# ZephirFXEC/HNanoSolver

Measured on AMD Instinct MI355X. Metric: solver substeps/sec (advect + 50 red-black SOR iterations + project) at N active voxels, higher is better.
Workload: dtype f32

## Files before the change

hnanosolver_amd/csrc/hns_advect.hip:

```cpp
#include <cstdlib>
#include <cstring>

#include "hns_device.hpp"

namespace hns {

struct Taps {
	int t[8];
	float fx, fy, fz;
};

constexpr unsigned kOutside = 0xFFFFE000u;
constexpr uint64_t kNarrowBytes = 0xFFFF0000ull;

__device__ __forceinline__ f3 ldv(const v4i& r, unsigned o4) {
	const v3f v = hns_buffer_load_v3f32(r, (int)(o4 + (o4 << 1)), 0, 0);
	return f3{v.x, v.y, v.z};
}
__device__ __forceinline__ float lds1(const v4i& r, unsigned o4) { return hns_buffer_load_f32(r, (int)o4, 0, 0); }

__device__ __forceinline__ void ld_zpair(const v4i& r, unsigned lo, unsigned hi, float& a, float& b) {
	const v2f32 v = hns_buffer_load_v2f32(r, (int)lo, 0, 0);
	a = v.x;
	b = v.y;
	if (hi != lo + 4u) b = lds1(r, hi);
}

struct GenericTabs {
	int nbr[27], base[27];
	__device__ __forceinline__ void set(int t, int nb) { nbr[t] = nb, base[t] = nb < 0 ? -1 : nb * 512; }
};
constexpr int kPadTab = 48;
struct NarrowTabs {
	int nbr[27];
	unsigned b4[27], b4p[kPadTab];
	__device__ __forceinline__ void set(int t, int nb) {
		const int ax = t / 9, ay = (t - 9 * ax) / 3, az = t - 9 * ax - 3 * ay;
		nbr[t] = nb, b4[t] = b4p[(ax * 4 + ay) * 4 + az] = nb < 0 ? kOutside : (unsigned)nb * 2048u;
	}
};

__device__ __forceinline__ int3 voxel_ijk(const int4 org, int n) { return int3{org.x + (n >> 6), org.y + ((n >> 3) & 7), org.z + (n & 7)}; }

template <class Tabs>
struct LeafVoxel {
	Tabs& tabs;
	const int n, leaf, idx;
	int4 org;
	int3 c;
	float px, py, pz;
	__device__ __forceinline__ LeafVoxel(const GridDev& g, Tabs& t) : tabs(t), n(threadIdx.x), leaf(launch_leaf(g, blockIdx.x)), idx(leaf * 512 + n) {}
	__device__ __forceinline__ void stage(const GridDev& g) {
		org = g.origins[leaf];
		if (threadIdx.x < 27) tabs.set(threadIdx.x, g.nbr27[leaf * 27 + threadIdx.x]);
		__syncthreads();
		c = voxel_ijk(org, n);
		px = (float)c.x, py = (float)c.y, pz = (float)c.z;
	}
};
typedef LeafVoxel<GenericTabs> GenericCtx;
typedef LeafVoxel<NarrowTabs> NarrowCtx;

__device__ __forceinline__ constexpr int tap_of(int q) { return ((q & 1) << 2) | (q & 2) | (q >> 2); }
template <int XS = 100, int YS = 10>
__device__ __forceinline__ constexpr int box_corner(int q) { return (q & 1) * XS + ((q >> 1) & 1) * YS + (q >> 2); }
__device__ __forceinline__ void tri_weights(float tx, float ty, float tz, float (&w)[8]) {
	const float itx = 1.0f - tx, ity = 1.0f - ty, itz = 1.0f - tz;
	const float w00 = itx * ity, w10 = tx * ity, w01 = itx * ty, w11 = tx * ty;
	w[0] = w00 * itz, w[1] = w10 * itz, w[2] = w01 * itz, w[3] = w11 * itz, w[4] = w00 * tz, w[5] = w10 * tz, w[6] = w01 * tz, w[7] = w11 * tz;
}
template <class T>
__device__ __forceinline__ T bfecc_limit(T phiOrig, const T (&nbr)[6], T phiForward, T phiCorr) {
	T mn = phiOrig, mx = phiOrig;
#pragma unroll
	for (int d = 0; d < 6; ++d) {
		mn = __builtin_elementwise_min(mn, nbr[d]);
		mx = __builtin_elementwise_max(mx, nbr[d]);
	}
	mn = __builtin_elementwise_min(mn, phiForward);
	mx = __builtin_elementwise_max(mx, phiForward);
	return __builtin_elementwise_max(mn, __builtin_elementwise_min(phiCorr, mx));
}
template <class Fetch>
__device__ __forceinline__ f3 bfecc_limit_v(const f3& vo, const f3& vf, const f3& vb, Fetch nbr) {
	float nx[6], ny[6], nz[6];
#pragma unroll
	for (int d = 0; d < 6; ++d) {
		const f3 t = nbr(d);
		nx[d] = t.x, ny[d] = t.y, nz[d] = t.z;
	}
	return f3{bfecc_limit(vo.x, nx, vf.x, vf.x + 0.5f * (vo.x - vb.x)), bfecc_limit(vo.y, ny, vf.y, vf.y + 0.5f * (vo.y - vb.y)),
	          bfecc_limit(vo.z, nz, vf.z, vf.z + 0.5f * (vo.z - vb.z))};
}

struct TapsB {
	unsigned o[8];
	float fx, fy, fz;
};

__device__ __forceinline__ Taps make_taps(const GridDev& g, const GenericCtx& C, float x, float y, float z) {
	Taps T;
	const int4 org = C.org;
	const int i = __float2int_rd(x), j = __float2int_rd(y), k = __float2int_rd(z);
	T.fx = x - (float)i;
	T.fy = y - (float)j;
	T.fz = z - (float)k;
	const int ax0 = (i >> 3) - (org.x >> 3) + 1, ax1 = ((i + 1) >> 3) - (org.x >> 3) + 1;
	const int ay0 = (j >> 3) - (org.y >> 3) + 1, ay1 = ((j + 1) >> 3) - (org.y >> 3) + 1;
	const int az0 = (k >> 3) - (org.z >> 3) + 1, az1 = ((k + 1) >> 3) - (org.z >> 3) + 1;
	const bool near = ((unsigned)ax0 <= 2u) & ((unsigned)ax1 <= 2u) & ((unsigned)ay0 <= 2u) & ((unsigned)ay1 <= 2u) & ((unsigned)az0 <= 2u) &
	                  ((unsigned)az1 <= 2u);
	if (near) {
		const int sx[2] = {ax0 * 9, ax1 * 9}, sy[2] = {ay0 * 3, ay1 * 3}, sz[2] = {az0, az1};
		const int lx[2] = {(i & 7) << 6, ((i + 1) & 7) << 6}, ly[2] = {(j & 7) << 3, ((j + 1) & 7) << 3}, lz[2] = {k & 7, (k + 1) & 7};
#pragma unroll
		for (int c = 0; c < 8; ++c) {
			const int di = c >> 2, dj = (c >> 1) & 1, dk = c & 1;
			const int b = C.tabs.base[sx[di] + sy[dj] + sz[dk]];
			T.t[c] = b < 0 ? -1 : b + (lx[di] | ly[dj] | lz[dk]);
		}
	} else {
		int any = 0;
		far_cell_taps(g, C.tabs.nbr, org, i, j, k, T.t);
#pragma unroll
		for (int c = 0; c < 8; ++c) any |= T.t[c];
		if (any < 0 && g.far_flag) *g.far_flag = 1;
	}
	return T;
}

__device__ __forceinline__ TapsB make_taps_b(const GridDev& g, const NarrowCtx& C, float x, float y, float z) {
	TapsB T;
	const int4 org = C.org;
	const int i = __float2int_rd(x), j = __float2int_rd(y), k = __float2int_rd(z);
	T.fx = x - (float)i;
	T.fy = y - (float)j;
	T.fz = z - (float)k;
	const unsigned dx = (unsigned)(i - (org.x - 8)), dy = (unsigned)(j - (org.y - 8)), dz = (unsigned)(k - (org.z - 8));
	if (max(dx, max(dy, dz)) < 23u) {
		const unsigned ex = dx + 1u, ey = dy + 1u, ez = dz + 1u;
		const unsigned X[2] = {(dx & 24u) << 3, (ex & 24u) << 3}, Y[2] = {(dy & 24u) << 1, (ey & 24u) << 1}, Z[2] = {(dz & 24u) >> 1, (ez & 24u) >> 1};
		const unsigned lx[2] = {(dx & 7u) << 8, (ex & 7u) << 8}, ly[2] = {(dy & 7u) << 5, (ey & 7u) << 5}, lz[2] = {(dz & 7u) << 2, (ez & 7u) << 2};
		const unsigned XY[4] = {X[0] | Y[0], X[0] | Y[1], X[1] | Y[0], X[1] | Y[1]};
		const unsigned lxy[4] = {lx[0] | ly[0], lx[0] | ly[1], lx[1] | ly[0], lx[1] | ly[1]};
		const char* tab = reinterpret_cast<const char*>(C.tabs.b4p);
#pragma unroll
		for (int c = 0; c < 8; ++c) {
			const int dij = c >> 1, dk = c & 1;
			T.o[c] = *reinterpret_cast<const unsigned*>(tab + (XY[dij] | Z[dk])) + lxy[dij] + lz[dk];
		}
	} else {
		int any = 0, ft[8];
		far_cell_taps(g, C.tabs.nbr, org, i, j, k, ft);
#pragma unroll
		for (int c = 0; c < 8; ++c) {
			any |= ft[c];
			T.o[c] = ft[c] < 0 ? kOutside : (unsigned)ft[c] << 2;
		}
		if (any < 0 && g.far_flag) *g.far_flag = 1;
	}
	return T;
}

__device__ __forceinline__ float ldz(const float* __restrict__ f, int idx) {
	const float v = f[idx < 0 ? 0 : idx];
	return idx < 0 ? 0.0f : v;
}

__device__ __forceinline__ float tri_f_t(const float* __restrict__ f, const Taps& T) {
	float c[8];
#pragma unroll
	for (int q = 0; q < 8; ++q) c[q] = ldz(f, T.t[q]);
	return tri_nest(c, T.fx, T.fy, T.fz, lerp_f);
}

__device__ __forceinline__ f3 tri_v_t(const float* __restrict__ u, const Taps& T) {
	float x[8], y[8], z[8];
#pragma unroll
	for (int q = 0; q < 8; ++q) {
		const f3 c = ld3z(u, T.t[q]);
		x[q] = c.x, y[q] = c.y, z[q] = c.z;
	}
	return f3{tri_nest(x, T.fx, T.fy, T.fz, lerp_c), tri_nest(y, T.fx, T.fy, T.fz, lerp_c), tri_nest(z, T.fx, T.fy, T.fz, lerp_c)};
}

struct V3 {
	v2f32 xy;
	float z;
};
__device__ __forceinline__ V3 lerp_v3(const V3& a, const V3& b, float w) {
	V3 r;
	r.xy = __builtin_elementwise_fma(v2f32{w, w}, b.xy - a.xy, a.xy);
	r.z = __fmaf_rn(w, b.z - a.z, a.z);
	return r;
}
__device__ __forceinline__ f3 tri_v_b(const v4i& ru, const TapsB& T) {
	V3 c[8];
#pragma unroll
	for (int q = 0; q < 8; ++q) {
		const v3f v = hns_buffer_load_v3f32(ru, (int)(T.o[q] + (T.o[q] << 1)), 0, 0);
		c[q].xy = v2f32{v.x, v.y};
		c[q].z = v.z;
	}
	const V3 r = tri_nest(c, T.fx, T.fy, T.fz, lerp_v3);
	return f3{r.xy.x, r.xy.y, r.z};
}

__device__ __forceinline__ float tri_f_b(const v4i& rf, const TapsB& T) {
	float c[8];
#pragma unroll
	for (int q = 0; q < 8; ++q) c[q] = lds1(rf, T.o[q]);
	return tri_nest(c, T.fx, T.fy, T.fz, lerp_f);
}

template <int AXIS, int DIR>
__device__ __forceinline__ int nbr_idx(const int* s_base, int leaf, int n) {
	constexpr int shift = AXIS == 0 ? 6 : (AXIS == 1 ? 3 : 0);
	constexpr int stride = 1 << shift;
	constexpr int dslot = AXIS == 0 ? 9 : (AXIS == 1 ? 3 : 1);
	const int c = (n >> shift) & 7;
	const bool inside = DIR > 0 ? c != 7 : c != 0;
	const int b = s_base[13 + DIR * dslot];
	const int in_leaf = leaf * 512 + n + DIR * stride;
	const int out_leaf = b < 0 ? -1 : b + n - DIR * 7 * stride;
	return inside ? in_leaf : out_leaf;
}

__device__ __forceinline__ void nbr6(const int* s_base, int leaf, int n, int (&t)[6]) {
	t[0] = nbr_idx<0, -1>(s_base, leaf, n);
	t[1] = nbr_idx<0, 1>(s_base, leaf, n);
	t[2] = nbr_idx<1, -1>(s_base, leaf, n);
	t[3] = nbr_idx<1, 1>(s_base, leaf, n);
	t[4] = nbr_idx<2, -1>(s_base, leaf, n);
	t[5] = nbr_idx<2, 1>(s_base, leaf, n);
}


__device__ __forceinline__ unsigned halo_off(const unsigned* s_b4, int h) {
	int slot, local;
	halo_entry(h, slot, local);
	return s_b4[slot] + ((unsigned)local << 2);
}

constexpr int kBox = 1000, kBoxShell = kBox - 512;
constexpr int kVY = 24, kVX = 10 * kVY, kVP = 10 * kVX;
template <int XS = 100, int YS = 10>
__device__ __forceinline__ void box_shell_entry(int h, int& slot, int& local, int& cell) {
	int bx, by, bz;
	if (h < 200) {
		const int side = h >= 100, r = h - 100 * side;
		bx = 9 * side, by = r / 10, bz = r - 10 * by;
	} else if (h < 360) {
		const int q = h - 200, side = q >= 80, r = q - 80 * side;
		bx = 1 + r / 10, by = 9 * side, bz = r - 10 * (bx - 1);
	} else {
		const int q = h - 360, side = q >> 6, r = q & 63;
		bx = 1 + (r >> 3), by = 1 + (r & 7), bz = 9 * side;
	}
	slot = ((bx + 7) >> 3) * 9 + ((by + 7) >> 3) * 3 + ((bz + 7) >> 3);
	local = (((bx + 7) & 7) << 6) | (((by + 7) & 7) << 3) | ((bz + 7) & 7);
	cell = bx * XS + by * YS + bz;
}
template <int XS = 100, int YS = 10>
__device__ __forceinline__ unsigned box_shell_off(const unsigned* s_b4, int h, int& cell) {
	unsigned off = 0u;
	cell = 0;
	if (h < kBoxShell) {
		int slot, local;
		box_shell_entry<XS, YS>(h, slot, local, cell);
		off = s_b4[slot] + ((unsigned)local << 2);
	}
	return off;
}
template <int XS = 100, int YS = 10>
__device__ __forceinline__ int box_own(int n) { return ((n >> 6) + 1) * XS + (((n >> 3) & 7) + 1) * YS + (n & 7) + 1; }
template <int XS = 100, int YS = 10>
__device__ __forceinline__ constexpr int box_nbr(int d) { return (d & 1 ? 1 : -1) * (d < 2 ? XS : (d < 4 ? YS : 1)); }

template <int XS, int YS, int PS>
__device__ __forceinline__ f3 velocity_box_load(float* s_box, const v4i& ru, int n, const f3& vo, unsigned off) {
	const int ob = box_own<XS, YS>(n);
	s_box[ob] = vo.x, s_box[ob + PS] = vo.y, s_box[ob + 2 * PS] = vo.z;
	f3 h = {0.0f, 0.0f, 0.0f};
	if (n < kBoxShell) h = ldv(ru, off);
	return h;
}
template <int PS>
__device__ __forceinline__ void velocity_box_store(float* s_box, int n, int cell, const f3& h) {
	if (n < kBoxShell) s_box[cell] = h.x, s_box[cell + PS] = h.y, s_box[cell + 2 * PS] = h.z;
}
__device__ __forceinline__ V3 box_v3(const float* s_box, int a) {
	V3 r;
	r.xy = v2f32{s_box[a], s_box[a + kVP]};
	r.z = s_box[a + 2 * kVP];
	return r;
}
__device__ __forceinline__ f3 box_f3(const float* s_box, int a) {
	const V3 t = box_v3(s_box, a);
	return f3{t.xy.x, t.xy.y, t.z};
}
__device__ __forceinline__ f3 tri_v_box(const float* s_box, int a, float fx, float fy, float fz) {
	V3 c[8];
#pragma unroll
	for (int q = 0; q < 8; ++q) c[q] = box_v3(s_box, a + box_corner<kVX, kVY>(tap_of(q)));
	const V3 r = tri_nest(c, fx, fy, fz, lerp_v3);
	return f3{r.xy.x, r.xy.y, r.z};
}
__device__ __forceinline__ f3 sample_velocity(const GridDev& g, const NarrowCtx& C, const v4i& ru, const float* s_box, float sx, float sy, float sz) {
	const int i = __float2int_rd(sx), j = __float2int_rd(sy), k = __float2int_rd(sz);
	const unsigned rx = (unsigned)(i - (C.org.x - 1)), ry = (unsigned)(j - (C.org.y - 1)), rz = (unsigned)(k - (C.org.z - 1));
	if (__all(max(rx, max(ry, rz)) <= 8u)) return tri_v_box(s_box, (int)(rx * (unsigned)kVX + ry * (unsigned)kVY + rz), sx - (float)i, sy - (float)j, sz - (float)k);
	return tri_v_b(ru, make_taps_b(g, C, sx, sy, sz));
}

__device__ __forceinline__ float sdf_box_load(float* s_sdf, const v4i& rs, int n, int ob, float own, unsigned off) {
	s_sdf[ob] = own;
	float h = 0.0f;
	if (n < kBoxShell) h = lds1(rs, off);
	return h;
}
__device__ __forceinline__ void sdf_box_store(float* s_sdf, int n, int cell, float h) {
	if (n < kBoxShell) s_sdf[cell] = h;
}
template <int XS, int YS>
__device__ __forceinline__ float tri_f_box(const float* s_f, int a, float fx, float fy, float fz) {
	float c[8];
#pragma unroll
	for (int q = 0; q < 8; ++q) c[q] = s_f[a + box_corner<XS, YS>(tap_of(q))];
	return tri_nest(c, fx, fy, fz, lerp_f);
}
template <int XS, int YS>
__device__ __forceinline__ f3 collide_velocity(const float* s_sdf, int ob, f3 vc, float inv_dx) {
	const float sv = s_sdf[ob];
	if (sv < 0.0f) {
		vc.x = vc.y = vc.z = 0.0f;
	} else if (sv < 0.1f) {
		float nb[6];
#pragma unroll
		for (int d = 0; d < 6; ++d) nb[d] = s_sdf[ob + box_nbr<XS, YS>(d)];
		vc = no_slip_blend(vc, sdf_normal_of(nb, inv_dx), 1.0f - (sv / 1.5f));
	}
	return vc;
}

template <bool COLL>
__device__ __forceinline__ void advect_vector_n(const GridDev& g, const float* __restrict__ u, float* __restrict__ out, const float* __restrict__ sdf, float* s_sdf, const float scaled_dt,
                                                const float inv_dx) {
	__shared__ NarrowTabs tabs;
	__shared__ float s_box[3 * kVP];
	NarrowCtx C(g, tabs);
	const v4i ru = field_rsrc(u, (unsigned)g.n_leaves * 6144u);
	const f3 vo = ldv(ru, (unsigned)C.idx << 2);
	v4i rs = {0, 0, 0, 0};
	float so = 0.0f;
	if constexpr (COLL) {
		rs = field_rsrc(sdf, (unsigned)g.n_leaves * 2048u);
		so = lds1(rs, (unsigned)C.idx << 2);
	}
	C.stage(g);
	int cell;
	const unsigned off = box_shell_off<kVX, kVY>(tabs.b4, C.n, cell);
	const int ob = box_own<kVX, kVY>(C.n);
	const f3 hv = velocity_box_load<kVX, kVY, kVP>(s_box, ru, C.n, vo, off);
	if constexpr (COLL) sdf_box_store(s_sdf, C.n, cell, sdf_box_load(s_sdf, rs, C.n, ob, so, off));
	velocity_box_store<kVP>(s_box, C.n, cell, hv);
	float sx = C.px - scaled_dt * vo.x, sy = C.py - scaled_dt * vo.y, sz = C.pz - scaled_dt * vo.z;
	float rx = C.px, ry = C.py, rz = C.pz;
	f3 vf = {0.0f, 0.0f, 0.0f}, vb = {0.0f, 0.0f, 0.0f};
	__syncthreads();
#pragma unroll 1
	for (int pass = 0; pass < 2; ++pass) {
		f3 v;
		if constexpr (COLL) {
			const int i = __float2int_rd(sx), j = __float2int_rd(sy), k = __float2int_rd(sz);
			const unsigned cx = (unsigned)(i - (C.org.x - 1)), cy = (unsigned)(j - (C.org.y - 1)), cz = (unsigned)(k - (C.org.z - 1));
			const bool boxed = __all(max(cx, max(cy, cz)) <= 8u);
			const int a = (int)(cx * (unsigned)kVX + cy * (unsigned)kVY + cz);
			float d;
			if (boxed)
				d = tri_f_box<kVX, kVY>(s_sdf, a, sx - (float)i, sy - (float)j, sz - (float)k);
			else
				d = tri_f_b(rs, make_taps_b(g, C, sx, sy, sz));
			if (d < 0.0f) sx = rx, sy = ry, sz = rz;
			v = sample_velocity(g, C, ru, s_box, sx, sy, sz);
		} else {
			v = sample_velocity(g, C, ru, s_box, sx, sy, sz);
		}
		if (pass == 0) {
			vf = v;
			if constexpr (COLL) rx = sx, ry = sy, rz = sz;
			sx = sx + scaled_dt * v.x, sy = sy + scaled_dt * v.y, sz = sz + scaled_dt * v.z;
		} else {
			vb = v;
		}
	}
	f3 vc = bfecc_limit_v(vo, vf, vb, [&](int d) { return box_f3(s_box, ob + box_nbr<kVX, kVY>(d)); });
	if constexpr (COLL) vc = collide_velocity<kVX, kVY>(s_sdf, ob, vc, inv_dx);
	st3(out, C.idx, vc);
}
__global__ __launch_bounds__(512) __attribute__((amdgpu_waves_per_eu(8, 8))) void k_advect_vector_n(const GridDev g, const float* __restrict__ u, float* __restrict__ out, const float scaled_dt) {
	advect_vector_n<false>(g, u, out, nullptr, nullptr, scaled_dt, 0.0f);
}
constexpr int kVectorCollLds = (3 * kVP + kVP) * 4 + (int)sizeof(NarrowTabs);
static_assert(kVectorCollLds <= 160 * 1024 / 4, "k_advect_vector_n<true>: four workgroups per CU no longer fit the LDS");
template <bool COLL>
__global__ __launch_bounds__(512) __attribute__((amdgpu_waves_per_eu(8, 8))) void k_advect_vector_n(const GridDev g, const float* __restrict__ u, float* __restrict__ out,
                                                                                                const float* __restrict__ sdf, const float scaled_dt, const float inv_dx) {
	static_assert(COLL, "without a collision field: the kernel of the same name that takes no SDF");
	__shared__ float s_sdf[kVP];
	advect_vector_n<true>(g, u, out, sdf, s_sdf, scaled_dt, inv_dx);
}

template <bool COLL>
__global__ __launch_bounds__(512) void k_advect_vector(const GridDev g, const float* __restrict__ u, float* __restrict__ out,
                                                       const float* __restrict__ sdf, const float scaled_dt, const float inv_dx) {
	__shared__ GenericTabs tabs;
	GenericCtx C(g, tabs);
	C.stage(g);
	const int idx = C.idx;

	const f3 vo = ld3(u, idx);
	float sx = C.px - scaled_dt * vo.x, sy = C.py - scaled_dt * vo.y, sz = C.pz - scaled_dt * vo.z;
	float rx = C.px, ry = C.py, rz = C.pz;
	f3 vf = {0.0f, 0.0f, 0.0f}, vb = {0.0f, 0.0f, 0.0f};
#pragma unroll 1
	for (int pass = 0; pass < 2; ++pass) {
		Taps T = make_taps(g, C, sx, sy, sz);
		if (COLL) {
			if (tri_f_t(sdf, T) < 0.0f) {
				sx = rx, sy = ry, sz = rz;
				T = make_taps(g, C, sx, sy, sz);
			}
		}
		const f3 v = tri_v_t(u, T);
		if (pass == 0) {
			vf = v;
			rx = sx, ry = sy, rz = sz;
			sx = sx + scaled_dt * v.x, sy = sy + scaled_dt * v.y, sz = sz + scaled_dt * v.z;
		} else {
			vb = v;
		}
	}
	int nb[6];
	nbr6(tabs.base, C.leaf, C.n, nb);
	f3 vc = bfecc_limit_v(vo, vf, vb, [&](int d) { return ld3z(u, nb[d]); });

	if (COLL) {
		const float sv = sdf[idx];
		if (sv < 0.0f) {
			vc.x = vc.y = vc.z = 0.0f;
		} else if (sv < 0.1f) {
			const f3 nrm = sdf_normal(g, tabs.nbr, C.org, sdf, C.c.x, C.c.y, C.c.z, inv_dx);
			vc = no_slip_blend(vc, nrm, 1.0f - (sv / 1.5f));
		}
	}
	st3(out, idx, vc);
}


__global__ __launch_bounds__(512) void k_advect_scalar_n(const GridDev g, const float* __restrict__ u, const float* __restrict__ in, float* __restrict__ out,
                                                         const float scaled_dt) {
	__shared__ NarrowTabs tabs;
	NarrowCtx C(g, tabs);
	C.stage(g);
	const int n = C.n;
	const unsigned bytes1 = (unsigned)g.n_leaves * 2048u, own = (unsigned)C.idx << 2;
	const v4i ru = field_rsrc(u, bytes1 * 3u), rf = field_rsrc(in, bytes1);

	__shared__ float s_tile[kTile];
	const float phiOrig = lds1(rf, own);
	s_tile[n] = phiOrig;
	if (n < 384) s_tile[512 + n] = lds1(rf, halo_off(tabs.b4, n));
	const f3 vc = ldv(ru, own);
	float sx = C.px - scaled_dt * vc.x, sy = C.py - scaled_dt * vc.y, sz = C.pz - scaled_dt * vc.z;
	float phiForward = 0.0f, phiBackward = 0.0f;
#pragma unroll 1
	for (int pass = 0; pass < 2; ++pass) {
		const TapsB T = make_taps_b(g, C, sx, sy, sz);
		const float phi = tri_f_b(rf, T);
		if (pass == 0) {
			phiForward = phi;
			const f3 vf = tri_v_b(ru, T);
			sx = sx + scaled_dt * vf.x, sy = sy + scaled_dt * vf.y, sz = sz + scaled_dt * vf.z;
		} else {
			phiBackward = phi;
		}
	}
	const float error = phiOrig - phiBackward;
	__syncthreads();
	const float nv[6] = {s_tile[tile_nbr<0, -1>(n)], s_tile[tile_nbr<0, 1>(n)], s_tile[tile_nbr<1, -1>(n)], s_tile[tile_nbr<1, 1>(n)], s_tile[tile_nbr<2, -1>(n)], s_tile[tile_nbr<2, 1>(n)]};
	out[C.idx] = bfecc_limit(phiOrig, nv, phiForward, phiForward + 0.5f * error);
}

template <bool COLL>
__global__ __launch_bounds__(512) void k_advect_scalar(const GridDev g, const float* __restrict__ u, const float* __restrict__ in,
                                                       float* __restrict__ out, const float* __restrict__ sdf, const float scaled_dt) {
	__shared__ GenericTabs tabs;
	GenericCtx C(g, tabs);
	C.stage(g);
	const int idx = C.idx;

	const float phiOrig = in[idx];
	const f3 vc = ld3(u, idx);
	float sx = C.px - scaled_dt * vc.x, sy = C.py - scaled_dt * vc.y, sz = C.pz - scaled_dt * vc.z;
	float rx = C.px, ry = C.py, rz = C.pz;
	float phiForward = 0.0f, phiBackward = 0.0f;
#pragma unroll 1
	for (int pass = 0; pass < 2; ++pass) {
		Taps T = make_taps(g, C, sx, sy, sz);
		if (COLL) {
			if (tri_f_t(sdf, T) < 0.0f) {
				sx = rx, sy = ry, sz = rz;
				T = make_taps(g, C, sx, sy, sz);
			}
		}
		const float phi = tri_f_t(in, T);
		if (pass == 0) {
			phiForward = phi;
			const f3 vf = tri_v_t(u, T);
			rx = sx, ry = sy, rz = sz;
			sx = sx + scaled_dt * vf.x, sy = sy + scaled_dt * vf.y, sz = sz + scaled_dt * vf.z;
		} else {
			phiBackward = phi;
		}
	}
	const float error = phiOrig - phiBackward;
	int nb[6];
	nbr6(tabs.base, C.leaf, C.n, nb);
	float nv[6];
#pragma unroll
	for (int d = 0; d < 6; ++d) nv[d] = ldz(in, nb[d]);
	out[idx] = bfecc_limit(phiOrig, nv, phiForward, phiForward + 0.5f * error);
}


#define HNS_MAX_SCALARS 8
struct ScalarPtrs {
	const float* in[HNS_MAX_SCALARS];
	float* out[HNS_MAX_SCALARS];
	int n;
	const float* q4;
	float* q4_out[4];
};

__device__ __forceinline__ float tri_f_zpair(const v4i& rf, const TapsB& T) {
	float c[8];
#pragma unroll
	for (int m = 0; m < 4; ++m) ld_zpair(rf, T.o[2 * m], T.o[2 * m + 1], c[2 * m], c[2 * m + 1]);
	return tri_nest(c, T.fx, T.fy, T.fz, lerp_f);
}
__global__ __launch_bounds__(512) __attribute__((amdgpu_waves_per_eu(8, 8))) void k_advect_scalar_multi_n(const GridDev g, const float* __restrict__ u, const ScalarPtrs P, const float scaled_dt) {
	__shared__ NarrowTabs tabs;
	NarrowCtx C(g, tabs);
	const int n = C.n;
	const unsigned bytes1 = (unsigned)g.n_leaves * 2048u, own = (unsigned)C.idx << 2;
	const v4i ru = field_rsrc(u, bytes1 * 3u);
	const f3 vc = ldv(ru, own);
	C.stage(g);
	float sx = C.px - scaled_dt * vc.x, sy = C.py - scaled_dt * vc.y, sz = C.pz - scaled_dt * vc.z;
	TapsB B, F;
#pragma unroll 1
	for (int pass = 0; pass < 2; ++pass) {
		F = make_taps_b(g, C, sx, sy, sz);
		if (pass == 0) {
			B = F;
			const f3 vf = tri_v_b(ru, B);
			sx = sx + scaled_dt * vf.x, sy = sy + scaled_dt * vf.y, sz = sz + scaled_dt * vf.z;
		}
	}
	const unsigned ho = n < 384 ? halo_off(tabs.b4, n) : 0u;
	__shared__ float s_tile[2][kTile];
	for (int s = 0; s < P.n; ++s) {
		const v4i rf = field_rsrc(P.in[s], bytes1);
		float* tile = s_tile[s & 1];
		const float phiOrig = lds1(rf, own);
		tile[n] = phiOrig;
		if (n < 384) tile[512 + n] = lds1(rf, ho);
		const float phiForward = tri_f_zpair(rf, B), phiBackward = tri_f_zpair(rf, F);
		const float error = phiOrig - phiBackward;
		__syncthreads();
		const float nv[6] = {tile[tile_nbr<0, -1>(n)], tile[tile_nbr<0, 1>(n)], tile[tile_nbr<1, -1>(n)], tile[tile_nbr<1, 1>(n)], tile[tile_nbr<2, -1>(n)], tile[tile_nbr<2, 1>(n)]};
		P.out[s][C.idx] = bfecc_limit(phiOrig, nv, phiForward, phiForward + 0.5f * error);
	}
}

__device__ __forceinline__ void interp_from_taps(const Taps& T, int oob, int (&ix)[8], float (&w)[8]) {
	tri_weights(T.fx, T.fy, T.fz, w);
#pragma unroll
	for (int q = 0; q < 8; ++q) ix[q] = T.t[tap_of(q)] < 0 ? oob : T.t[tap_of(q)];
}
__device__ __forceinline__ void add_weighted(f3& a, const f3& v, float w) { a.x = a.x + w * v.x, a.y = a.y + w * v.y, a.z = a.z + w * v.z; }

template <bool BOX>
__device__ __forceinline__ bool sample_setup(const GridDev& g, const NarrowCtx& C, float x, float y, float z, unsigned oob4, int& cell, unsigned (&o)[8], float (&w)[8]) {
	const int i = __float2int_rd(x), j = __float2int_rd(y), k = __float2int_rd(z);
	const unsigned rx = (unsigned)(i - (C.org.x - 1)), ry = (unsigned)(j - (C.org.y - 1)), rz = (unsigned)(k - (C.org.z - 1));
	const bool boxed = BOX && max(rx, max(ry, rz)) <= 8u;
	cell = boxed ? (int)((rx * 10u + ry) * 10u + rz) : 0;
	float tx, ty, tz;
	if (boxed) {
		tx = x - (float)i, ty = y - (float)j, tz = z - (float)k;
#pragma unroll
		for (int q = 0; q < 8; ++q) o[q] = 0u;
	} else {
		const TapsB T = make_taps_b(g, C, x, y, z);
		tx = T.fx, ty = T.fy, tz = T.fz;
#pragma unroll
		for (int q = 0; q < 8; ++q) o[q] = T.o[tap_of(q)] >= kOutside ? oob4 : T.o[tap_of(q)];
	}
	tri_weights(tx, ty, tz, w);
	return boxed;
}

__device__ __forceinline__ bool sdf_hit(const GridDev& g, const NarrowCtx& C, const v4i& rs, const float* s_sdf, float x, float y, float z) {
	const int i = __float2int_rd(x), j = __float2int_rd(y), k = __float2int_rd(z);
	const unsigned rx = (unsigned)(i - (C.org.x - 1)), ry = (unsigned)(j - (C.org.y - 1)), rz = (unsigned)(k - (C.org.z - 1));
	float d;
	if (max(rx, max(ry, rz)) <= 8u)
		d = tri_f_box<100, 10>(s_sdf, (int)((rx * 10u + ry) * 10u + rz), x - (float)i, y - (float)j, z - (float)k);
	else
		d = tri_f_b(rs, make_taps_b(g, C, x, y, z));
	return d < 0.0f;
}
template <bool Q4, bool AHEAD, bool COLL>
__device__ __forceinline__ void advect_scalars_n(const GridDev& g, const float* __restrict__ u, const ScalarPtrs& P, const float scaled_dt, float* __restrict__ adv_out,
                                                 const float* __restrict__ sdf) {
	static_assert(!(Q4 && AHEAD), "the look-ahead form is float-only");
	static_assert(!(AHEAD && COLL), "with a collider the next substep rewrites the velocity before it advects it: nothing to look ahead to");
	__shared__ NarrowTabs tabs;
	NarrowCtx C(g, tabs);
	const int n = C.n, idx = C.idx;
	const unsigned bytes1 = (unsigned)g.n_leaves * 2048u;
	const v4i ru = field_rsrc(u, bytes1 * 3u);
	const unsigned own = (unsigned)idx << 2, oob4 = (unsigned)g.oob << 2;
	const f3 vc = ldv(ru, own);
	v4i rs = {0, 0, 0, 0};
	float so = 0.0f;
	if constexpr (COLL) {
		rs = field_rsrc(sdf, bytes1);
		so = lds1(rs, own);
	}
	C.stage(g);

	const int ob = box_own(n);
	int hcell;
	unsigned ho = box_shell_off(tabs.b4, n, hcell);
	__shared__ float s_sdf[COLL ? kBox : 1];
	if constexpr (COLL) sdf_box_store(s_sdf, n, hcell, sdf_box_load(s_sdf, rs, n, ob, so, ho));
	ho = ho >= kOutside ? oob4 : ho;
	constexpr bool FIRST = Q4;
	__shared__ float s_ubox[FIRST ? 3 * kBox : 1];
	if constexpr (FIRST) velocity_box_store<kBox>(s_ubox, n, hcell, velocity_box_load<100, 10, kBox>(s_ubox, ru, n, vc, ho));

	float bx = C.px - scaled_dt * vc.x, by = C.py - scaled_dt * vc.y, bz = C.pz - scaled_dt * vc.z;
	__shared__ float s_back[COLL && FIRST ? 3 * 512 : 1];
	if constexpr (COLL) {
		__syncthreads();
		if (sdf_hit(g, C, rs, s_sdf, bx, by, bz)) bx = C.px, by = C.py, bz = C.pz;
		if constexpr (FIRST) s_back[n] = bx, s_back[n + 512] = by, s_back[n + 1024] = bz;
		asm volatile("" : "+v"(bx), "+v"(by), "+v"(bz));
	}
	unsigned bo[8], fo[8];
	float bw[8], fw[8];
	bool bboxed = false;
	int ba = 0;
	f3 vf = {0.0f, 0.0f, 0.0f};
	__shared__ float s_vbox[AHEAD ? 3 * kVP : 1];
	__shared__ float s_wf[AHEAD ? 3 * 512 : 1];
	if constexpr (AHEAD) {
		int vcell;
		const unsigned voff = box_shell_off<kVX, kVY>(tabs.b4, n, vcell);
		const f3 hv = velocity_box_load<kVX, kVY, kVP>(s_vbox, ru, n, vc, voff);
		const TapsB T = make_taps_b(g, C, bx, by, bz);
		V3 c[8];
#pragma unroll
		for (int q = 0; q < 8; ++q) {
			const v3f v = hns_buffer_load_v3f32(ru, (int)(T.o[tap_of(q)] + (T.o[tap_of(q)] << 1)), 0, 0);
			c[tap_of(q)].xy = v2f32{v.x, v.y};
			c[tap_of(q)].z = v.z;
		}
		const float* __restrict__ uoob = u + 3 * (size_t)g.oob;
		const f3 uo = {uoob[0], uoob[1], uoob[2]};
		velocity_box_store<kVP>(s_vbox, n, vcell, hv);
		tri_weights(T.fx, T.fy, T.fz, bw);
		V3 z[4];
#pragma unroll
		for (int q = 0; q < 8; ++q) {
			const int t = tap_of(q);
			const bool outside = T.o[t] >= kOutside;
			bo[q] = outside ? oob4 : T.o[t];
			add_weighted(vf, f3{outside ? uo.x : c[t].xy.x, outside ? uo.y : c[t].xy.y, outside ? uo.z : c[t].z}, bw[q]);
			if (t & 1) z[t >> 1] = lerp_v3(c[t - 1], c[t], T.fz);
		}
		const V3 r = tri_nest_yx(z, T.fx, T.fy, lerp_v3);
		s_wf[n] = r.xy.x, s_wf[n + 512] = r.xy.y, s_wf[n + 1024] = r.z;
	} else {
		bboxed = sample_setup<FIRST>(g, C, bx, by, bz, oob4, ba, bo, bw);
		f3 vt[8];
		if (!bboxed) {
#pragma unroll
			for (int q = 0; q < 8; ++q) vt[q] = ldv(ru, bo[q]);
		}
		if constexpr (FIRST && !COLL) __syncthreads();
		if (bboxed) {
#pragma unroll
			for (int q = 0; q < 8; ++q) {
				const int a = ba + box_corner(q);
				vt[q] = f3{s_ubox[a], s_ubox[a + kBox], s_ubox[a + 2 * kBox]};
			}
		}
#pragma unroll
		for (int q = 0; q < 8; ++q) add_weighted(vf, vt[q], bw[q]);
	}
	int fa;
	float fx = bx + scaled_dt * vf.x, fy = by + scaled_dt * vf.y, fz = bz + scaled_dt * vf.z;
	if constexpr (COLL) {
		if (sdf_hit(g, C, rs, s_sdf, fx, fy, fz)) {
			if constexpr (FIRST) {
				int m = n;
				asm volatile("" : "+v"(m));
				fx = s_back[m], fy = s_back[m + 512], fz = s_back[m + 1024];
			} else {
				fx = bx, fy = by, fz = bz;
			}
		}
	}
	const bool boxed = sample_setup<true>(g, C, fx, fy, fz, oob4, fa, fo, fw);
	constexpr bool SHARE = COLL && Q4;
	if constexpr (SHARE) {
		if (bboxed) bo[0] = (unsigned)ba;
		if (boxed) fo[0] = (unsigned)fa;
		asm volatile("" : "+v"(bo[0]), "+v"(fo[0]));
	}
	const int bcell = SHARE ? (int)bo[0] : ba, fcell = SHARE ? (int)fo[0] : fa;
	__shared__ float s_box[2][kBox];
	if constexpr (Q4) {
		__shared__ v4f32 s_box4[kBox];
		const v4i rq = field_rsrc(P.q4, bytes1 * 4u);
		const v4f32 phiOrig = hns_buffer_load_v4f32(rq, (int)(own << 2), 0, 0);
		s_box4[ob] = phiOrig;
		if (n < kBoxShell) s_box4[hcell] = hns_buffer_load_v4f32(rq, (int)(ho << 2), 0, 0);
		v4f32 phiF = {0.0f, 0.0f, 0.0f, 0.0f}, phiB = {0.0f, 0.0f, 0.0f, 0.0f};
		if (!bboxed) {
			v4f32 c[8];
#pragma unroll
			for (int q = 0; q < 8; ++q) c[q] = hns_buffer_load_v4f32(rq, (int)(bo[q] << 2), 0, 0);
#pragma unroll
			for (int q = 0; q < 8; ++q) phiF = __builtin_elementwise_fma(c[q], v4f32{bw[q], bw[q], bw[q], bw[q]}, phiF);
		}
		if (!boxed) {
			v4f32 c[8];
#pragma unroll
			for (int q = 0; q < 8; ++q) c[q] = hns_buffer_load_v4f32(rq, (int)(fo[q] << 2), 0, 0);
#pragma unroll
			for (int q = 0; q < 8; ++q) phiB = __builtin_elementwise_fma(c[q], v4f32{fw[q], fw[q], fw[q], fw[q]}, phiB);
		}
		__syncthreads();
		if (bboxed) {
#pragma unroll
			for (int q = 0; q < 8; ++q) phiF = __builtin_elementwise_fma(s_box4[bcell + box_corner(q)], v4f32{bw[q], bw[q], bw[q], bw[q]}, phiF);
		}
		if (boxed) {
#pragma unroll
			for (int q = 0; q < 8; ++q) phiB = __builtin_elementwise_fma(s_box4[fcell + box_corner(q)], v4f32{fw[q], fw[q], fw[q], fw[q]}, phiB);
		}
		v4f32 nv[6];
#pragma unroll
		for (int d = 0; d < 6; ++d) nv[d] = s_box4[ob + box_nbr(d)];
		const v4f32 r = bfecc_limit(phiOrig, nv, phiF, __builtin_elementwise_fma(v4f32{0.5f, 0.5f, 0.5f, 0.5f}, phiOrig - phiB, phiF));
		P.q4_out[0][idx] = r.x, P.q4_out[1][idx] = r.y, P.q4_out[2][idx] = r.z, P.q4_out[3][idx] = r.w;
	}
	for (int s = 0; s < P.n; ++s) {
		const v4i rf = field_rsrc(P.in[s], bytes1);
		float* box = s_box[s & 1];
		const float phiOrig = lds1(rf, own);
		box[ob] = phiOrig;
		if (n < kBoxShell) box[hcell] = lds1(rf, ho);
		float vb[8], vf8[8];
		if (!bboxed) {
#pragma unroll
			for (int q = 0; q < 4; ++q) ld_zpair(rf, bo[q], bo[q + 4], vb[q], vb[q + 4]);
		}
		if (!boxed) {
#pragma unroll
			for (int q = 0; q < 4; ++q) ld_zpair(rf, fo[q], fo[q + 4], vf8[q], vf8[q + 4]);
		}
		float phiF = 0.0f, phiB = 0.0f;
		__syncthreads();
		if (bboxed) {
#pragma unroll
			for (int q = 0; q < 8; ++q) vb[q] = box[bcell + box_corner(q)];
		}
#pragma unroll
		for (int q = 0; q < 8; ++q) phiF = __fmaf_rn(vb[q], bw[q], phiF);
		if (boxed) {
#pragma unroll
			for (int q = 0; q < 8; ++q) vf8[q] = box[fcell + box_corner(q)];
		}
#pragma unroll
		for (int q = 0; q < 8; ++q) phiB = __fmaf_rn(vf8[q], fw[q], phiB);
		float nv[6];
#pragma unroll
		for (int d = 0; d < 6; ++d) nv[d] = box[ob + box_nbr(d)];
		P.out[s][idx] = bfecc_limit(phiOrig, nv, phiF, __fmaf_rn(0.5f, phiOrig - phiB, phiF));
	}
	if constexpr (AHEAD) {
		__syncthreads();
		int m = n;
		asm volatile("" : "+v"(m));
		const int obv = box_own<kVX, kVY>(m);
		const int3 w = voxel_ijk(C.org, m);
		const f3 vo = box_f3(s_vbox, obv);
		const f3 wf = f3{s_wf[m], s_wf[m + 512], s_wf[m + 1024]};
		const float cx = (float)w.x - scaled_dt * vo.x, cy = (float)w.y - scaled_dt * vo.y, cz = (float)w.z - scaled_dt * vo.z;
		const f3 wb = sample_velocity(g, C, ru, s_vbox, cx + scaled_dt * wf.x, cy + scaled_dt * wf.y, cz + scaled_dt * wf.z);
		st3(adv_out, idx, bfecc_limit_v(vo, wf, wb, [&](int d) { return box_f3(s_vbox, obv + box_nbr<kVX, kVY>(d)); }));
	}
}

template <bool Q4, bool AHEAD = false>
__global__ __launch_bounds__(512) __attribute__((amdgpu_waves_per_eu(Q4 || AHEAD ? 6 : 4))) void k_advect_scalars_n(const GridDev g, const float* __restrict__ u, const ScalarPtrs P, const float scaled_dt,
                                                                                                            float* __restrict__ adv_out) {
	advect_scalars_n<Q4, AHEAD, false>(g, u, P, scaled_dt, adv_out, nullptr);
}
constexpr int kScalarsQ4CollLds = (int)sizeof(NarrowTabs) + (3 * kBox + 2 * kBox + 4 * kBox + kBox + 3 * 512) * 4;
static_assert(kScalarsQ4CollLds <= 160 * 1024 / 3, "k_advect_scalars_n<true, false, true>: three workgroups per CU no longer fit the LDS");
template <bool Q4, bool AHEAD, bool COLL>
__global__ __launch_bounds__(512) __attribute__((amdgpu_waves_per_eu(Q4 ? 6 : 4))) void k_advect_scalars_n(const GridDev g, const float* __restrict__ u, const ScalarPtrs P, const float* __restrict__ sdf,
                                                                                                   const float scaled_dt) {
	static_assert(COLL && !AHEAD, "without a collision field: the kernel of the same name that takes no SDF");
	advect_scalars_n<Q4, false, true>(g, u, P, scaled_dt, nullptr, sdf);
}

template <bool COLL>
__global__ __launch_bounds__(512) void k_advect_scalars(const GridDev g, const float* __restrict__ u, const ScalarPtrs P,
                                                        const float* __restrict__ sdf, const float scaled_dt) {
	__shared__ GenericTabs tabs;
	GenericCtx C(g, tabs);
	C.stage(g);
	const int idx = C.idx;

	const f3 vc = ld3(u, idx);
	float sx = C.px - scaled_dt * vc.x, sy = C.py - scaled_dt * vc.y, sz = C.pz - scaled_dt * vc.z;
	float rx = C.px, ry = C.py, rz = C.pz;
	int bi[8], fi[8];
	float bw[8], fw[8];
#pragma unroll 1
	for (int pass = 0; pass < 2; ++pass) {
		Taps T = make_taps(g, C, sx, sy, sz);
		if (COLL) {
			if (tri_f_t(sdf, T) < 0.0f) {
				sx = rx, sy = ry, sz = rz;
				T = make_taps(g, C, sx, sy, sz);
			}
		}
		if (pass == 0) {
			interp_from_taps(T, g.oob, bi, bw);
			f3 vf = {0.0f, 0.0f, 0.0f};
#pragma unroll
			for (int q = 0; q < 8; ++q) add_weighted(vf, ld3(u, bi[q]), bw[q]);
			rx = sx, ry = sy, rz = sz;
			sx = sx + scaled_dt * vf.x, sy = sy + scaled_dt * vf.y, sz = sz + scaled_dt * vf.z;
		} else {
			interp_from_taps(T, g.oob, fi, fw);
		}
	}
	int nb[6];
	nbr6(tabs.base, C.leaf, C.n, nb);
#pragma unroll
	for (int d = 0; d < 6; ++d) nb[d] = nb[d] < 0 ? g.oob : nb[d];
	for (int s = 0; s < P.n; ++s) {
		const float* __restrict__ in = P.in[s];
		const float phiOrig = in[idx];
		float phiF = 0.0f, phiB = 0.0f;
#pragma unroll
		for (int q = 0; q < 8; ++q) {
			phiF = __fmaf_rn(in[bi[q]], bw[q], phiF);
			phiB = __fmaf_rn(in[fi[q]], fw[q], phiB);
		}
		float nv[6];
#pragma unroll
		for (int d = 0; d < 6; ++d) nv[d] = in[nb[d]];
		P.out[s][idx] = bfecc_limit(phiOrig, nv, phiF, __fmaf_rn(0.5f, phiOrig - phiB, phiF));
	}
}

}

using namespace hns;

static bool narrow_fields(const hns_grid* g) {
	return !options().advect_generic.load() && (uint64_t)g->topo.n_leaves * 6144u <= hns::kNarrowBytes;
}

enum class AdvectForm { collision, narrow_collision, narrow, generic };
static AdvectForm advect_form(const hns_grid* g, const float* sdf, int has_collision) {
	if (has_collision && sdf) return narrow_fields(g) && !options().collide_generic.load() ? AdvectForm::narrow_collision : AdvectForm::collision;
	return narrow_fields(g) ? AdvectForm::narrow : AdvectForm::generic;
}
static const char* advect_vector_kernel(AdvectForm f) {
	switch (f) {
	case AdvectForm::collision: return "k_advect_vector<true>";
	case AdvectForm::narrow_collision: return "k_advect_vector_n<coll>";
	case AdvectForm::narrow: return "k_advect_vector_n";
	default: return "k_advect_vector<false>";
	}
}
static const char* advect_scalars_kernel(AdvectForm f) {
	switch (f) {
	case AdvectForm::collision: return "k_advect_scalars<true>";
	case AdvectForm::narrow_collision: return "k_advect_scalars_n<coll>";
	case AdvectForm::narrow: return "k_advect_scalars_n";
	default: return "k_advect_scalars<false>";
	}
}

static GridDev reversed(const hns_grid* g) {
	GridDev gd = g->dev();
	gd.rev = 1;
	return gd;
}

static int fill_scalar_ptrs(ScalarPtrs& P, const float* const* in, float* const* out, int n) {
	int bad = -1;
	P.n = n;
	P.q4 = nullptr, P.q4_out[0] = P.q4_out[1] = P.q4_out[2] = P.q4_out[3] = nullptr;
	for (int s = 0; s < HNS_MAX_SCALARS; ++s) {
		P.in[s] = s < n ? in[s] : nullptr;
		P.out[s] = s < n ? out[s] : nullptr;
		if (s < n && (!P.in[s] || !P.out[s]) && bad < 0) bad = s;
	}
	return bad;
}

extern "C" {

int hns_dev_advect_vector(hns_grid* g, const float* vel3, float* out3, const float* sdf, int has_collision, float dt, float inv_dx, void* stream) {
	if (int rc = check_grid(g, "hns_dev_advect_vector")) return rc;
	NULLCHK(!vel3 || !out3, "hns_dev_advect_vector");
	if (vel3 == out3) return fail(HNS_ERR_INVALID_ARGUMENT, "hns_dev_advect_vector: output must not alias input");
	if (g->n_active == 0) return HNS_OK;
	const float scaled_dt = dt * inv_dx;
	const dim3 grid((unsigned)g->n_active), block(512);
	switch (advect_form(g, sdf, has_collision)) {
	case AdvectForm::collision: hipLaunchKernelGGL(k_advect_vector<true>, grid, block, 0, (hipStream_t)stream, g->dev(), vel3, out3, sdf, scaled_dt, inv_dx); break;
	case AdvectForm::narrow_collision: hipLaunchKernelGGL(k_advect_vector_n<true>, grid, block, 0, (hipStream_t)stream, g->dev(), vel3, out3, sdf, scaled_dt, inv_dx); break;
	case AdvectForm::narrow: hipLaunchKernelGGL(k_advect_vector_n, grid, block, 0, (hipStream_t)stream, g->dev(), vel3, out3, scaled_dt); break;
	case AdvectForm::generic: hipLaunchKernelGGL(k_advect_vector<false>, grid, block, 0, (hipStream_t)stream, g->dev(), vel3, out3, sdf, scaled_dt, inv_dx); break;
	}
	return launch_status("hns_dev_advect_vector");
}

int hns_dev_advect_scalar(hns_grid* g, const float* vel3, const float* in, float* out, const float* sdf, int has_collision, float dt, float inv_dx,
                          void* stream) {
	if (int rc = check_grid(g, "hns_dev_advect_scalar")) return rc;
	NULLCHK(!vel3 || !in || !out, "hns_dev_advect_scalar");
	if (g->n_active == 0) return HNS_OK;
	const float scaled_dt = dt * inv_dx;
	const dim3 grid((unsigned)g->n_active), block(512);
	switch (advect_form(g, sdf, has_collision)) {
	case AdvectForm::narrow_collision:
	case AdvectForm::collision: hipLaunchKernelGGL(k_advect_scalar<true>, grid, block, 0, (hipStream_t)stream, g->dev(), vel3, in, out, sdf, scaled_dt); break;
	case AdvectForm::narrow: hipLaunchKernelGGL(k_advect_scalar_n, grid, block, 0, (hipStream_t)stream, g->dev(), vel3, in, out, scaled_dt); break;
	case AdvectForm::generic: hipLaunchKernelGGL(k_advect_scalar<false>, grid, block, 0, (hipStream_t)stream, g->dev(), vel3, in, out, sdf, scaled_dt); break;
	}
	return launch_status("hns_dev_advect_scalar");
}

int hns_dev_advect_scalars(hns_grid* g, const float* vel3, const float* const* in, float* const* out, int n, const float* sdf, int has_collision,
                           float dt, float inv_dx, void* stream) {
	if (int rc = check_grid(g, "hns_dev_advect_scalars")) return rc;
	NULLCHK(!vel3 || (n > 0 && (!in || !out)), "hns_dev_advect_scalars");
	if (g->n_active == 0 || n <= 0) return HNS_OK;
	const float scaled_dt = dt * inv_dx;
	const dim3 grid((unsigned)g->n_active), block(512);
	for (int base = 0; base < n; base += HNS_MAX_SCALARS) {
		ScalarPtrs P;
		const int bad = fill_scalar_ptrs(P, in + base, out + base, n - base < HNS_MAX_SCALARS ? n - base : HNS_MAX_SCALARS);
		if (bad >= 0) {
			set_error("hns_dev_advect_scalars: null device pointer for field %d", base + bad);
			return HNS_ERR_INVALID_ARGUMENT;
		}
		switch (advect_form(g, sdf, has_collision)) {
		case AdvectForm::collision: hipLaunchKernelGGL(k_advect_scalars<true>, grid, block, 0, (hipStream_t)stream, g->dev(), vel3, P, sdf, scaled_dt); break;
		case AdvectForm::narrow_collision: hipLaunchKernelGGL((k_advect_scalars_n<false, false, true>), grid, block, 0, (hipStream_t)stream, reversed(g), vel3, P, sdf, scaled_dt); break;
		case AdvectForm::narrow: hipLaunchKernelGGL(k_advect_scalars_n<false>, grid, block, 0, (hipStream_t)stream, reversed(g), vel3, P, scaled_dt, (float*)nullptr); break;
		case AdvectForm::generic: hipLaunchKernelGGL(k_advect_scalars<false>, grid, block, 0, (hipStream_t)stream, g->dev(), vel3, P, sdf, scaled_dt); break;
		}
	}
	return launch_status("hns_dev_advect_scalars");
}

int hns_dev_advect_scalar_multi(hns_grid* g, const float* vel3, const float* const* in, float* const* out, int n, const float* sdf, int has_collision, float dt, float inv_dx,
                                void* stream) {
	if (int rc = check_grid(g, "hns_dev_advect_scalar_multi")) return rc;
	NULLCHK(!vel3 || (n > 0 && (!in || !out)), "hns_dev_advect_scalar_multi");
	for (int i = 0; i < n; ++i) {
		if (!in[i] || !out[i]) {
			set_error("hns_dev_advect_scalar_multi: null device pointer for field %d", i);
			return HNS_ERR_INVALID_ARGUMENT;
		}
		if (out[i] == vel3) {
			set_error("hns_dev_advect_scalar_multi: output of field %d aliases the velocity", i);
			return HNS_ERR_INVALID_ARGUMENT;
		}
		for (int j = 0; j < n; ++j) {
			if (out[i] == in[j]) {
				set_error("hns_dev_advect_scalar_multi: output of field %d aliases the input of field %d", i, j);
				return HNS_ERR_INVALID_ARGUMENT;
			}
			if (j < i && out[i] == out[j]) {
				set_error("hns_dev_advect_scalar_multi: output of field %d is the output of field %d", i, j);
				return HNS_ERR_INVALID_ARGUMENT;
			}
		}
	}
	if (g->n_active == 0 || n <= 0) return HNS_OK;
	const float scaled_dt = dt * inv_dx;
	const dim3 grid((unsigned)g->n_active), block(512);
	const AdvectForm form = advect_form(g, sdf, has_collision);
	if (form == AdvectForm::narrow) {
		for (int base = 0; base < n; base += HNS_MAX_SCALARS) {
			const int m = n - base < HNS_MAX_SCALARS ? n - base : HNS_MAX_SCALARS;
			if (m == 1) {
				hipLaunchKernelGGL(k_advect_scalar_n, grid, block, 0, (hipStream_t)stream, g->dev(), vel3, in[base], out[base], scaled_dt);
				continue;
			}
			ScalarPtrs P;
			fill_scalar_ptrs(P, in + base, out + base, m);
			hipLaunchKernelGGL(k_advect_scalar_multi_n, grid, block, 0, (hipStream_t)stream, g->dev(), vel3, P, scaled_dt);
		}
	} else {
		for (int i = 0; i < n; ++i) {
			if (form == AdvectForm::collision || form == AdvectForm::narrow_collision)
				hipLaunchKernelGGL(k_advect_scalar<true>, grid, block, 0, (hipStream_t)stream, g->dev(), vel3, in[i], out[i], sdf, scaled_dt);
			else
				hipLaunchKernelGGL(k_advect_scalar<false>, grid, block, 0, (hipStream_t)stream, g->dev(), vel3, in[i], out[i], sdf, scaled_dt);
		}
	}
	return launch_status("hns_dev_advect_scalar_multi");
}

bool hns_advect_ahead_ok(const hns_grid* g) { return narrow_fields(g); }

int hns_dev_advect_scalars_ahead(hns_grid* g, const float* vel3, const float* const* in, float* const* out, int n, float* adv_out3, float dt, float inv_dx, void* stream) {
	if (int rc = check_grid(g, "hns_dev_advect_scalars_ahead")) return rc;
	NULLCHK(!vel3 || !adv_out3 || (n > 0 && (!in || !out)), "hns_dev_advect_scalars_ahead");
	if (vel3 == adv_out3) return fail(HNS_ERR_INVALID_ARGUMENT, "hns_dev_advect_scalars_ahead: adv_out3 must not alias vel3");
	if (n < 0 || n > HNS_MAX_SCALARS) return fail(HNS_ERR_INVALID_ARGUMENT, "hns_dev_advect_scalars_ahead: between 0 and 8 fields");
	if (!narrow_fields(g)) return fail(HNS_ERR_INVALID_ARGUMENT, "hns_dev_advect_scalars_ahead: grid too large for 32-bit offsets (or option advect = generic)");
	if (g->n_active == 0) return HNS_OK;
	ScalarPtrs P;
	const int bad = fill_scalar_ptrs(P, in, out, n);
	if (bad >= 0) {
		set_error("hns_dev_advect_scalars_ahead: null device pointer for field %d", bad);
		return HNS_ERR_INVALID_ARGUMENT;
	}
	hipLaunchKernelGGL((k_advect_scalars_n<false, true>), dim3((unsigned)g->n_active), dim3(512), 0, (hipStream_t)stream, reversed(g), vel3, P, dt * inv_dx, adv_out3);
	return launch_status("hns_dev_advect_scalars_ahead");
}

int hns_advect_scalars_q4(hns_grid* g, const float* vel3, const float* q4, float* const* q4_out, const float* const* in, float* const* out, int n, const float* sdf, float dt,
                          float inv_dx, void* stream) {
	if (int rc = check_grid(g, "hns_advect_scalars_q4")) return rc;
	NULLCHK(!vel3 || !q4 || !q4_out || (n > 0 && (!in || !out)), "hns_advect_scalars_q4");
	if (!hns_advect_q4_ok(g) || n > HNS_MAX_SCALARS) return fail(HNS_ERR_INVALID_ARGUMENT, "hns_advect_scalars_q4: grid too large for 32-bit offsets, or too many fields");
	if (g->n_active == 0) return HNS_OK;
	for (int c = 0; c < 4; ++c) NULLCHK(!q4_out[c], "hns_advect_scalars_q4");
	ScalarPtrs P;
	NULLCHK(fill_scalar_ptrs(P, in, out, n) >= 0, "hns_advect_scalars_q4");
	P.q4 = q4;
	for (int c = 0; c < 4; ++c) P.q4_out[c] = q4_out[c];
	if (sdf)
		hipLaunchKernelGGL((k_advect_scalars_n<true, false, true>), dim3((unsigned)g->n_active), dim3(512), 0, (hipStream_t)stream, reversed(g), vel3, P, sdf, dt * inv_dx);
	else
		hipLaunchKernelGGL(k_advect_scalars_n<true>, dim3((unsigned)g->n_active), dim3(512), 0, (hipStream_t)stream, reversed(g), vel3, P, dt * inv_dx, (float*)nullptr);
	return launch_status("hns_advect_scalars_q4");
}
const char* hns_advect_scalars_q4_kernel(const float* sdf) { return sdf ? "k_advect_scalars_n<q4,coll>" : "k_advect_scalars_n<q4>"; }

const char* hns_advect_vector_kernel(const hns_grid* g, const float* sdf, int has_collision) { return advect_vector_kernel(advect_form(g, sdf, has_collision)); }
const char* hns_advect_scalars_kernel(const hns_grid* g, const float* sdf, int has_collision) { return advect_scalars_kernel(advect_form(g, sdf, has_collision)); }
const char* hns_advect_scalars_ahead_kernel(void) { return "k_advect_scalars_n<ahead>"; }

bool hns_advect_q4_ok(const hns_grid* g) { return narrow_fields(g) && (uint64_t)g->topo.n_leaves * 8192u <= hns::kNarrowBytes; }

}
```

Before: 658.2.

## Interleave velocity box components to shrink LDS and raise look-ahead advect occupancy

Stores the y component of the shared velocity box in the unused half of each padded y row, which cuts the box from three planes to two and shrinks LDS use for the vector and look-ahead advect kernels. The look-ahead scalar kernel now targets eight waves per EU, with a static_assert that four workgroups per CU fit in LDS. It also reads the grid struct straight from the kernarg segment, which is meant to keep fewer grid values live in registers. The risks are LDS bank conflicts from the new interleaved addressing and register spills under the tighter waves-per-EU cap.

```diff
diff --git a/hnanosolver_amd/csrc/hns_advect.hip b/hnanosolver_amd/csrc/hns_advect.hip
--- a/hnanosolver_amd/csrc/hns_advect.hip
+++ b/hnanosolver_amd/csrc/hns_advect.hip
@@ -244,6 +244,8 @@
 
 constexpr int kBox = 1000, kBoxShell = kBox - 512;
 constexpr int kVY = 24, kVX = 10 * kVY, kVP = 10 * kVX;
+constexpr int kVCy = kVY / 2, kVCz = kVP, kVBox = 2 * kVP;
+static_assert(kVCy + 10 <= kVY, "velocity box: the y rows (10 floats from kVCy) run into the next x row");
 template <int XS = 100, int YS = 10>
 __device__ __forceinline__ void box_shell_entry(int h, int& slot, int& local, int& cell) {
 	int bx, by, bz;
@@ -277,22 +279,22 @@
 template <int XS = 100, int YS = 10>
 __device__ __forceinline__ constexpr int box_nbr(int d) { return (d & 1 ? 1 : -1) * (d < 2 ? XS : (d < 4 ? YS : 1)); }
 
-template <int XS, int YS, int PS>
+template <int XS, int YS, int CY, int CZ>
 __device__ __forceinline__ f3 velocity_box_load(float* s_box, const v4i& ru, int n, const f3& vo, unsigned off) {
 	const int ob = box_own<XS, YS>(n);
-	s_box[ob] = vo.x, s_box[ob + PS] = vo.y, s_box[ob + 2 * PS] = vo.z;
+	s_box[ob] = vo.x, s_box[ob + CY] = vo.y, s_box[ob + CZ] = vo.z;
 	f3 h = {0.0f, 0.0f, 0.0f};
 	if (n < kBoxShell) h = ldv(ru, off);
 	return h;
 }
-template <int PS>
+template <int CY, int CZ>
 __device__ __forceinline__ void velocity_box_store(float* s_box, int n, int cell, const f3& h) {
-	if (n < kBoxShell) s_box[cell] = h.x, s_box[cell + PS] = h.y, s_box[cell + 2 * PS] = h.z;
+	if (n < kBoxShell) s_box[cell] = h.x, s_box[cell + CY] = h.y, s_box[cell + CZ] = h.z;
 }
 __device__ __forceinline__ V3 box_v3(const float* s_box, int a) {
 	V3 r;
-	r.xy = v2f32{s_box[a], s_box[a + kVP]};
-	r.z = s_box[a + 2 * kVP];
+	r.xy = v2f32{s_box[a], s_box[a + kVCy]};
+	r.z = s_box[a + kVCz];
 	return r;
 }
 __device__ __forceinline__ f3 box_f3(const float* s_box, int a) {
@@ -347,7 +349,7 @@
 __device__ __forceinline__ void advect_vector_n(const GridDev& g, const float* __restrict__ u, float* __restrict__ out, const float* __restrict__ sdf, float* s_sdf, const float scaled_dt,
                                                 const float inv_dx) {
 	__shared__ NarrowTabs tabs;
-	__shared__ float s_box[3 * kVP];
+	__shared__ float s_box[kVBox];
 	NarrowCtx C(g, tabs);
 	const v4i ru = field_rsrc(u, (unsigned)g.n_leaves * 6144u);
 	const f3 vo = ldv(ru, (unsigned)C.idx << 2);
@@ -361,9 +363,9 @@
 	int cell;
 	const unsigned off = box_shell_off<kVX, kVY>(tabs.b4, C.n, cell);
 	const int ob = box_own<kVX, kVY>(C.n);
-	const f3 hv = velocity_box_load<kVX, kVY, kVP>(s_box, ru, C.n, vo, off);
+	const f3 hv = velocity_box_load<kVX, kVY, kVCy, kVCz>(s_box, ru, C.n, vo, off);
 	if constexpr (COLL) sdf_box_store(s_sdf, C.n, cell, sdf_box_load(s_sdf, rs, C.n, ob, so, off));
-	velocity_box_store<kVP>(s_box, C.n, cell, hv);
+	velocity_box_store<kVCy, kVCz>(s_box, C.n, cell, hv);
 	float sx = C.px - scaled_dt * vo.x, sy = C.py - scaled_dt * vo.y, sz = C.pz - scaled_dt * vo.z;
 	float rx = C.px, ry = C.py, rz = C.pz;
 	f3 vf = {0.0f, 0.0f, 0.0f}, vb = {0.0f, 0.0f, 0.0f};
@@ -401,7 +403,7 @@
 __global__ __launch_bounds__(512) __attribute__((amdgpu_waves_per_eu(8, 8))) void k_advect_vector_n(const GridDev g, const float* __restrict__ u, float* __restrict__ out, const float scaled_dt) {
 	advect_vector_n<false>(g, u, out, nullptr, nullptr, scaled_dt, 0.0f);
 }
-constexpr int kVectorCollLds = (3 * kVP + kVP) * 4 + (int)sizeof(NarrowTabs);
+constexpr int kVectorCollLds = (kVBox + kVP) * 4 + (int)sizeof(NarrowTabs);
 static_assert(kVectorCollLds <= 160 * 1024 / 4, "k_advect_vector_n<true>: four workgroups per CU no longer fit the LDS");
 template <bool COLL>
 __global__ __launch_bounds__(512) __attribute__((amdgpu_waves_per_eu(8, 8))) void k_advect_vector_n(const GridDev g, const float* __restrict__ u, float* __restrict__ out,
@@ -622,11 +624,14 @@
 		d = tri_f_b(rs, make_taps_b(g, C, x, y, z));
 	return d < 0.0f;
 }
+__device__ __forceinline__ const GridDev& kernarg_grid() { return *reinterpret_cast<const GridDev*>((const void*)__builtin_amdgcn_kernarg_segment_ptr()); }
+
 template <bool Q4, bool AHEAD, bool COLL>
 __device__ __forceinline__ void advect_scalars_n(const GridDev& g, const float* __restrict__ u, const ScalarPtrs& P, const float scaled_dt, float* __restrict__ adv_out,
                                                  const float* __restrict__ sdf) {
 	static_assert(!(Q4 && AHEAD), "the look-ahead form is float-only");
 	static_assert(!(AHEAD && COLL), "with a collider the next substep rewrites the velocity before it advects it: nothing to look ahead to");
+	const GridDev& gk = AHEAD ? kernarg_grid() : g;
 	__shared__ NarrowTabs tabs;
 	NarrowCtx C(g, tabs);
 	const int n = C.n, idx = C.idx;
@@ -650,7 +655,7 @@
 	ho = ho >= kOutside ? oob4 : ho;
 	constexpr bool FIRST = Q4;
 	__shared__ float s_ubox[FIRST ? 3 * kBox : 1];
-	if constexpr (FIRST) velocity_box_store<kBox>(s_ubox, n, hcell, velocity_box_load<100, 10, kBox>(s_ubox, ru, n, vc, ho));
+	if constexpr (FIRST) velocity_box_store<kBox, 2 * kBox>(s_ubox, n, hcell, velocity_box_load<100, 10, kBox, 2 * kBox>(s_ubox, ru, n, vc, ho));
 
 	float bx = C.px - scaled_dt * vc.x, by = C.py - scaled_dt * vc.y, bz = C.pz - scaled_dt * vc.z;
 	__shared__ float s_back[COLL && FIRST ? 3 * 512 : 1];
@@ -665,13 +670,13 @@
 	bool bboxed = false;
 	int ba = 0;
 	f3 vf = {0.0f, 0.0f, 0.0f};
-	__shared__ float s_vbox[AHEAD ? 3 * kVP : 1];
+	__shared__ float s_vbox[AHEAD ? kVBox : 1];
 	__shared__ float s_wf[AHEAD ? 3 * 512 : 1];
 	if constexpr (AHEAD) {
 		int vcell;
 		const unsigned voff = box_shell_off<kVX, kVY>(tabs.b4, n, vcell);
-		const f3 hv = velocity_box_load<kVX, kVY, kVP>(s_vbox, ru, n, vc, voff);
-		const TapsB T = make_taps_b(g, C, bx, by, bz);
+		const f3 hv = velocity_box_load<kVX, kVY, kVCy, kVCz>(s_vbox, ru, n, vc, voff);
+		const TapsB T = make_taps_b(gk, C, bx, by, bz);
 		V3 c[8];
 #pragma unroll
 		for (int q = 0; q < 8; ++q) {
@@ -681,7 +686,7 @@
 		}
 		const float* __restrict__ uoob = u + 3 * (size_t)g.oob;
 		const f3 uo = {uoob[0], uoob[1], uoob[2]};
-		velocity_box_store<kVP>(s_vbox, n, vcell, hv);
+		velocity_box_store<kVCy, kVCz>(s_vbox, n, vcell, hv);
 		tri_weights(T.fx, T.fy, T.fz, bw);
 		V3 z[4];
 #pragma unroll
@@ -695,7 +700,7 @@
 		const V3 r = tri_nest_yx(z, T.fx, T.fy, lerp_v3);
 		s_wf[n] = r.xy.x, s_wf[n + 512] = r.xy.y, s_wf[n + 1024] = r.z;
 	} else {
-		bboxed = sample_setup<FIRST>(g, C, bx, by, bz, oob4, ba, bo, bw);
+		bboxed = sample_setup<FIRST>(gk, C, bx, by, bz, oob4, ba, bo, bw);
 		f3 vt[8];
 		if (!bboxed) {
 #pragma unroll
@@ -725,7 +730,7 @@
 			}
 		}
 	}
-	const bool boxed = sample_setup<true>(g, C, fx, fy, fz, oob4, fa, fo, fw);
+	const bool boxed = sample_setup<true>(gk, C, fx, fy, fz, oob4, fa, fo, fw);
 	constexpr bool SHARE = COLL && Q4;
 	if constexpr (SHARE) {
 		if (bboxed) bo[0] = (unsigned)ba;
@@ -813,13 +818,15 @@
 		const f3 vo = box_f3(s_vbox, obv);
 		const f3 wf = f3{s_wf[m], s_wf[m + 512], s_wf[m + 1024]};
 		const float cx = (float)w.x - scaled_dt * vo.x, cy = (float)w.y - scaled_dt * vo.y, cz = (float)w.z - scaled_dt * vo.z;
-		const f3 wb = sample_velocity(g, C, ru, s_vbox, cx + scaled_dt * wf.x, cy + scaled_dt * wf.y, cz + scaled_dt * wf.z);
+		const f3 wb = sample_velocity(gk, C, ru, s_vbox, cx + scaled_dt * wf.x, cy + scaled_dt * wf.y, cz + scaled_dt * wf.z);
 		st3(adv_out, idx, bfecc_limit_v(vo, wf, wb, [&](int d) { return box_f3(s_vbox, obv + box_nbr<kVX, kVY>(d)); }));
 	}
 }
 
+constexpr int kLookaheadLds = (int)sizeof(NarrowTabs) + (kVBox + 3 * 512 + 2 * kBox) * 4;
+static_assert(kLookaheadLds <= 160 * 1024 / 4, "k_advect_scalars_n<false, true>: four workgroups per CU no longer fit the LDS");
 template <bool Q4, bool AHEAD = false>
-__global__ __launch_bounds__(512) __attribute__((amdgpu_waves_per_eu(Q4 || AHEAD ? 6 : 4))) void k_advect_scalars_n(const GridDev g, const float* __restrict__ u, const ScalarPtrs P, const float scaled_dt,
+__global__ __launch_bounds__(512) __attribute__((amdgpu_waves_per_eu(AHEAD ? 8 : (Q4 ? 6 : 4), 8))) void k_advect_scalars_n(const GridDev g, const float* __restrict__ u, const ScalarPtrs P, const float scaled_dt,
                                                                                                             float* __restrict__ adv_out) {
 	advect_scalars_n<Q4, AHEAD, false>(g, u, P, scaled_dt, adv_out, nullptr);
 }
```

Measured after the change: 666.7 (median of 6 runs). 1.01x the previous value.
